# ucla-vision/xivo

Hardware: AMD Instinct MI355X
Metric: EKF updates/sec (state dim 250, 80 feats) @1 GPU; % MFMA roofline (higher is better)
Workload: dtype f64; 1 GPU; MH gating + UpdateJosephForm: state dim 250, 80 features (M=160), XIVO row sparsity, P/H/inn/R resident in HBM; filters_per_gpu=16384, global_batch=16384, parallelism=replicas x1 (no collective), pipeline=sparse-H (row-pair compressed H, whitened in-solve Joseph form), hand_over=dense H -> row-pair compressed rows every step, inside the timed region, route=sparse_in_solve, not_spd_filters=0

## Files before the change

### xivo_amd/csrc/trsm_lds_kernel.h

```cpp
#pragma once
#include <stdlib.h>
#include <stdio.h>

#include "mfma_util.h"

#ifndef XIVO_TRACE
#define XIVO_TRACE 0
#endif
#if XIVO_TRACE
__device__ unsigned long long xivo_trace_buf[512 * 32];
__device__ unsigned long long xivo_trace2_buf[128 * 16 * 4 * 16];
#define XTR(i) do { if (T4 && !WOUT && threadIdx.x == 0 && (blockIdx.x & 63) == 0 && (blockIdx.x >> 6) < 512) \
    xivo_trace_buf[(blockIdx.x >> 6) * 32 + (i)] = __builtin_amdgcn_s_memtime(); } while (0)
#define XTRP(i) do { if (FIXUP && threadIdx.x == 0 && (blockIdx.x & 63) == 0 && (blockIdx.x >> 6) < 512) \
    xivo_trace_buf[(blockIdx.x >> 6) * 32 + (i)] = __builtin_amdgcn_s_memtime(); } while (0)
#define XTR2(ph, slot) do { if (FIXUP && (threadIdx.x & 63) == 0 && (blockIdx.x & 63) == 0 && (blockIdx.x >> 6) < 128 && (ph) < 4 && (slot) < 16) \
    xivo_trace2_buf[(((blockIdx.x >> 6) * 16 + (threadIdx.x >> 6)) * 4 + (ph)) * 16 + (slot)] = __builtin_amdgcn_s_memtime(); } while (0)
extern "C" int xivo_hip_debug_read_trace(unsigned long long* out, int n) {
  return (int)hipMemcpyFromSymbol(out, HIP_SYMBOL(xivo_trace_buf), (size_t)n * sizeof(unsigned long long));
}
extern "C" int xivo_hip_debug_read_trace2(unsigned long long* out, int n) {
  return (int)hipMemcpyFromSymbol(out, HIP_SYMBOL(xivo_trace2_buf), (size_t)n * sizeof(unsigned long long));
}
#else
#define XTR(i) do {} while (0)
#define XTRP(i) do {} while (0)
#define XTR2(ph, slot) do {} while (0)
#endif

namespace xivo_hip {

namespace {

typedef unsigned int bufu2 __attribute__((ext_vector_type(2)));
__device__ __forceinline__ __amdgpu_buffer_rsrc_t buf_rsrc(const void* p) {
  return __builtin_amdgcn_make_buffer_rsrc(const_cast<void*>(p), 0, 0x7FFFFFFF, 0x00020000);
}
__device__ __forceinline__ double buf_ld(__amdgpu_buffer_rsrc_t r, unsigned voff, unsigned soff) {
  return __builtin_bit_cast(double, __builtin_amdgcn_raw_buffer_load_b64(r, voff, soff, 0));
}
__device__ __forceinline__ double buf_ld_once(__amdgpu_buffer_rsrc_t r, unsigned voff, unsigned soff) {
  return __builtin_bit_cast(double, __builtin_amdgcn_raw_buffer_load_b64(r, voff, soff, 0));
}
__device__ __forceinline__ void buf_st_f32(float v, __amdgpu_buffer_rsrc_t r, unsigned voff, unsigned soff) {
  __builtin_amdgcn_raw_buffer_store_b32(__builtin_bit_cast(unsigned, v), r, voff, soff, 0);
}
__device__ __forceinline__ void buf_st(double v, __amdgpu_buffer_rsrc_t r, unsigned voff, unsigned soff) {
  __builtin_amdgcn_raw_buffer_store_b64(__builtin_bit_cast(bufu2, v), r, voff, soff, 0);
}
__device__ __forceinline__ void buf_st_out(double v, __amdgpu_buffer_rsrc_t r, unsigned voff, unsigned soff) {
  __builtin_amdgcn_raw_buffer_store_b64(__builtin_bit_cast(bufu2, v), r, voff, soff, 0);
}

template <int NBM, bool SRC_REGS = false, bool NEG_OUT = false, bool FIXUP = false, bool YREGS = false, int NWV = 16>
__device__ __forceinline__ void sym_tiles_from_regs(const d4 (&X)[NBM], const d4 (&Wr)[NBM], double* sL, const double* __restrict__ Src, int ldsrc,
                                                    const double* __restrict__ Minit, int ldm, double* __restrict__ Out, int ldo,
                                                    int nb, int nwl, int jbp, bool live, int w, int wave, int lane) {
  const int li = lane & 15, lg = lane >> 4;
  const int nph = (nwl + jbp - 1) / jbp;
  const int bufsz = jbp * nb * 256;
  auto issue = [&](int p) {
    const int jb0 = p * jbp, nj = min(jbp, nwl - jb0);
    double* buf = sL + (p & 1) * bufsz;
    if (SRC_REGS) {
      if (live && w >= jb0 && w < jb0 + nj) {
        double* dst = buf + (w - jb0) * nb * 256 + lane;
#pragma unroll
        for (int mb = 0; mb < NBM; ++mb) {
          if (mb < nb) {
#pragma unroll
            for (int r = 0; r < 4; ++r) dst[(mb * 4 + r) * 64] = YREGS ? fma(2.0, Wr[mb][r], -X[mb][r]) : X[mb][r];
          }
        }
      }
      return;
    }
    for (int q = wave; q < nj * 2 * nb; q += NWV) {
      const int jl = q / (2 * nb), t = q - jl * 2 * nb;
      const double* src = Src + (16 * (jb0 + jl) + 2 * (lane & 7)) + (long)(8 * t + (lane >> 3)) * ldsrc;
      __builtin_amdgcn_global_load_lds((const __attribute__((address_space(1))) void*)src,
                                       (__attribute__((address_space(3))) void*)(buf + jl * nb * 256 + t * 128), 16, 0, 0);
    }
  };
  auto my_tiles = [&](int p) -> unsigned {
    unsigned todo = 0;
    if (!live || p >= nph) return todo;
    const int jb0 = p * jbp, nj = min(jbp, nwl - jb0);
    for (int jl = 0; jl < nj; ++jl) {
      int d = w - (jb0 + jl);
      if (d < 0) d += nwl;
      if (2 * d < nwl || (2 * d == nwl && w > jb0 + jl)) todo |= 1u << jl;
    }
    return todo;
  };
  const __amdgpu_buffer_rsrc_t rM = buf_rsrc(Minit), rO = buf_rsrc(Out);
  const unsigned vM = (unsigned)(li + lg * ldm) * 8u;
  const unsigned vO = (unsigned)(li + lg * ldo) * 8u, vOt = (unsigned)(lg + li * ldo) * 8u;
  auto load_m = [&](int jb, d4& acc) {
    const int ba = jb <= w ? w : jb, bb = jb <= w ? jb : w;
#pragma unroll
    for (int r = 0; r < 4; ++r)
      acc[r] = buf_ld_once(rM, vM, (unsigned)(16 * ba + (16 * bb + 4 * r) * ldm) * 8u);
  };
  issue(0);
  unsigned todo = my_tiles(0);
  d4 nxt = d4{0.0, 0.0, 0.0, 0.0};
  if (todo) load_m(__builtin_ctz(todo), nxt);
  for (int p = 0; p < nph; ++p) {
    XTRP(8 + 3 * p);
    asm volatile("s_waitcnt vmcnt(0)" ::: "memory");
    XTRP(9 + 3 * p);
    __syncthreads();
    XTRP(10 + 3 * p);
    XTR2(p, 0);
    int tslot = 2;
    const int jb0 = p * jbp;
    const double* buf = sL + (p & 1) * bufsz;
    if (FIXUP) {
      if (live && w >= jb0 && w < jb0 + min(jbp, nwl - jb0)) {
        double* dst = sL + (p & 1) * bufsz + (w - jb0) * nb * 256 + lane;
#pragma unroll
        for (int mb = 0; mb < NBM; ++mb) {
          if (mb < nb) {
#pragma unroll
            for (int r = 0; r < 4; ++r) dst[(mb * 4 + r) * 64] = fma(2.0, dst[(mb * 4 + r) * 64], -X[mb][r]);
          }
        }
      }
      lds_barrier();
    }
    XTR2(p, 1);
    bool fetch = p + 1 < nph;
    while (todo) {
      const int jl = __builtin_ctz(todo);
      todo &= todo - 1;
      const int jb = jb0 + jl;
      d4 acc = -nxt;
      if (fetch) { asm volatile("" : "+v"(acc[0]), "+v"(acc[1]), "+v"(acc[2]), "+v"(acc[3])); issue(p + 1); fetch = false; }
      if (todo) load_m(jb0 + __builtin_ctz(todo), nxt);
      const double* Bop = buf + jl * nb * 256 + lane;
      if (jb <= w) {
#pragma unroll
        for (int mb = 0; mb < NBM; ++mb) {
          if (mb < nb) {
#pragma unroll
            for (int r = 0; r < 4; ++r) acc = mfma(Bop[(mb * 4 + r) * 64], X[mb][r], acc);
          }
        }
      } else {
#pragma unroll
        for (int mb = 0; mb < NBM; ++mb) {
          if (mb < nb) {
#pragma unroll
            for (int r = 0; r < 4; ++r) acc = mfma(X[mb][r], Bop[(mb * 4 + r) * 64], acc);
          }
        }
      }
      XTR2(p, tslot); ++tslot;
      const int ba = jb <= w ? w : jb, bbk = jb <= w ? jb : w;
      const int a = 16 * ba + li, b = 16 * bbk + lg;
#pragma unroll
      for (int r = 0; r < 4; ++r) {
        const int bb = b + 4 * r;
        if (jb != w || a >= bb) {
          const double v = NEG_OUT ? -acc[r] : acc[r];
          buf_st_out(v, rO, vO, (unsigned)(16 * ba + (16 * bbk + 4 * r) * ldo) * 8u);
          if (a != bb) buf_st_out(v, rO, vOt, (unsigned)(16 * bbk + 4 * r + 16 * ba * ldo) * 8u);
        }
      }
      XTR2(p, tslot); ++tslot;
    }
    XTR2(p, 14);
    if (fetch) issue(p + 1);
    todo = my_tiles(p + 1);
    if (todo) load_m((p + 1) * jbp + __builtin_ctz(todo), nxt);
  }
  XTRP(8 + 3 * nph);
}

template <int NBM, int TF, int NWV = 16, int MINB = 1>
__global__ __launch_bounds__(64 * NWV, MINB) void trsm_lds_f64_kernel(TrsmArgs g) {
  constexpr int BLK = 16 * 17;
  constexpr int NT = 64 * NWV;
  static_assert(TF != 3, "TF == 3 (the round-2 expanded Joseph form) was removed in round 6");
  constexpr bool T4 = TF == 4 || TF == 5;
  constexpr bool WOUT = TF == 5;
  constexpr bool KEEPW = T4 && (NBM <= 6 || (NBM == 7 && NWV <= 12 && MINB <= 3));
  constexpr bool PACK = T4 && NBM > 10;
  extern __shared__ __attribute__((aligned(16))) double sL[];
  const int chunks = (g.Np + 16 * NWV - 1) / (16 * NWV);
  const int b = blockIdx.x;
  const int xcd = b & 7, slot = b >> 3;
  const int filt = (slot / chunks) * 8 + xcd;
  const int chunk = slot % chunks;
  if (filt >= g.batch) return;
  const int tid = threadIdx.x, lane = tid & 63, wave = __builtin_amdgcn_readfirstlane(tid >> 6);
  const int li = lane & 15, lg = lane >> 4;
  const int nb = g.Mp / 16;
  const double* __restrict__ LU = g.LU + (long)filt * g.strideLU;
  const double* __restrict__ invD = g.invD + (long)filt * g.strideInvD;
  const double* __restrict__ PHT = g.PHT + (long)filt * g.stridePHT;
  const long ld = g.ldlu;

  XTR(0);
  const int c0 = chunk * 16 * NWV + wave * 16;
  const bool live = c0 < g.Np;
  const __amdgpu_buffer_rsrc_t rPHT = buf_rsrc(PHT), rK = buf_rsrc(g.K + (long)filt * g.strideK),
                               rInn = buf_rsrc(g.fwd_only ? g.y + (long)filt * g.strideY : g.inn + (long)filt * g.strideInn);
  const unsigned vPHT = (unsigned)((c0 + li) + lg * g.ldpht) * 8u;
  const unsigned vK = (unsigned)((c0 + li) + lg * g.ldk) * 8u;
  d4 X[NBM];
  auto load_rhs = [&](int i0, int i1) {
#pragma unroll
    for (int i = 0; i < NBM; ++i) {
      if (i >= i0 && i < i1) {
        X[i] = d4{0.0, 0.0, 0.0, 0.0};
        if (live && i < nb) {
#pragma unroll
          for (int r = 0; r < 4; ++r) X[i][r] = buf_ld_once(rPHT, vPHT, (unsigned)((16 * i + 4 * r) * g.ldpht) * 8u);
        }
      }
    }
  };
  load_rhs(0, NBM);
  d4 Wk[KEEPW ? NBM : 1];
#pragma unroll
  for (int i = 0; i < (KEEPW ? NBM : 1); ++i) Wk[i] = d4{0.0, 0.0, 0.0, 0.0};

  const int nblk = nb * (nb + 1) / 2;
  constexpr bool DIAG = !PACK && T4;
  constexpr int CPY = (NBM * (NBM + 1) / 2 * 128 + NT - 1) / NT;
  constexpr int CPD = DIAG ? (NBM * 128 + NT - 1) / NT : 0;
  constexpr int CPB = 4;
  double* sD = sL + nblk * BLK;
#pragma unroll
  for (int u0 = 0; u0 < CPY + CPD; u0 += CPB) {
    d2 cv[CPB], cu[CPB];
#pragma unroll
    for (int q = 0; q < CPB; ++q) {
      const int u = u0 + q;
      cv[q] = d2{0.0, 0.0}; cu[q] = d2{0.0, 0.0};
      if (u < CPY) {
        const int e = tid + NT * u;
        if (e < nblk * 128) {
          const int t = e >> 7, w = e & 127;
          int i = 0;
          while ((i + 1) * (i + 2) / 2 <= t) ++i;
          const int k = t - i * (i + 1) / 2;
          const int r = (w & 7) * 2, c = w >> 3;
          cv[q] = *reinterpret_cast<const d2*>(i != k ? LU + (16 * i + r) + (long)(16 * k + c) * ld : invD + (long)k * 512 + r + 16 * c);
          if (PACK && i == k) { cu[q][0] = LU[(16 * k + c) + (long)(16 * k + r) * ld]; cu[q][1] = LU[(16 * k + c) + (long)(16 * k + r + 1) * ld]; }
        }
      } else if (u < CPY + CPD) {
        const int e = tid + NT * (u - CPY);
        if (e < nb * 128) {
          const int k = e >> 7, w = e & 127;
          cv[q] = *reinterpret_cast<const d2*>(LU + (16 * k + (w & 7) * 2) + (long)(16 * k + (w >> 3)) * ld);
        }
      }
    }
#pragma unroll
    for (int q = 0; q < CPB; ++q) {
      const int u = u0 + q;
      if (u < CPY) {
        const int e = tid + NT * u;
        if (e < nblk * 128) {
          const int t = e >> 7, w = e & 127;
          int i = 0;
          while ((i + 1) * (i + 2) / 2 <= t) ++i;
          const int k = t - i * (i + 1) / 2;
          const int r = (w & 7) * 2, c = w >> 3;
          d2 v = cv[q];
          if (PACK && i == k) { v[0] = r >= c ? v[0] : cu[q][0]; v[1] = r + 1 >= c ? v[1] : cu[q][1]; }
          sL[t * BLK + r + 17 * c] = v[0];
          sL[t * BLK + r + 1 + 17 * c] = v[1];
        }
      } else if (u < CPY + CPD) {
        const int e = tid + NT * (u - CPY);
        if (e < nb * 128) {
          const int k = e >> 7, w = e & 127;
          const int r = (w & 7) * 2, c = w >> 3;
          sD[k * BLK + r + 17 * c] = r >= c ? cv[q][0] : 0.0;
          sD[k * BLK + r + 1 + 17 * c] = r + 1 >= c ? cv[q][1] : 0.0;
        }
      }
    }
    __builtin_amdgcn_sched_barrier(0);
  }
  if (PACK) {
    for (int e = tid; e < nb * 16; e += NT) {
      const int k = e >> 4, c = e & 15;
      sL[(k * (k + 1) / 2 + k) * BLK + 16 + 17 * c] = LU[(16 * k + c) + (long)(16 * k + c) * ld];
    }
  }
  XTR(1);
  __syncthreads();
  XTR(2);
  if (!TF && !live) return;
  if (live) {
#pragma unroll
  for (int k = 0; k < NBM; ++k) {
    if (k < nb) {
      const double* Dk = sL + (k * (k + 1) / 2 + k) * BLK;
      d4 t = d4{0.0, 0.0, 0.0, 0.0};
#pragma unroll
      for (int s = 0; s < 4; ++s) {
        double a = Dk[li + 17 * (4 * s + lg)];
        if (PACK) a = li >= 4 * s + lg ? a : 0.0;
        t = mfma(a, X[k][s], t);
      }
      X[k] = t;
#pragma unroll
      for (int s = 0; s < 4; ++s) {
#pragma unroll
        for (int i = k + 1; i < NBM; ++i) {
          if (i < nb) {
            const double a = sL[(i * (i + 1) / 2 + k) * BLK + li + 17 * (4 * s + lg)];
            X[i] = mfma(-a, t[s], X[i]);
          }
        }
      }
    }
  }
  XTR(3);
  double part = 0.0;
  if (KEEPW) {
#pragma unroll
    for (int i = 0; i < NBM; ++i) Wk[i] = X[i];
  }
  if (T4 && !KEEPW) {
#pragma unroll
    for (int i = 0; i < NBM; ++i) {
      if (i < nb) {
#pragma unroll
        for (int r = 0; r < 4; ++r) buf_st(X[i][r], rK, vK, (unsigned)((16 * i + 4 * r) * g.ldk) * 8u);
      }
    }
  }
  XTR(4);
#pragma unroll
  for (int k = NBM - 1; k >= 0; --k) {
    if (k < nb && !g.fwd_only) {
      const double* Dk = sL + (k * (k + 1) / 2 + k) * BLK;
      d4 wk = d4{0.0, 0.0, 0.0, 0.0};
      if (KEEPW) wk = Wk[k];
      else if (T4) {
        if (k == nb - 1) wk = X[k];
        else {
#pragma unroll
          for (int r = 0; r < 4; ++r) wk[r] = buf_ld(rK, vK, (unsigned)((16 * k + 4 * r) * g.ldk) * 8u);
        }
      }
      d4 t = d4{0.0, 0.0, 0.0, 0.0};
#pragma unroll
      for (int s = 0; s < 4; ++s) {
        double a = Dk[(4 * s + lg) + 17 * li];
        if (PACK) a = 4 * s + lg >= li ? a : 0.0;
        t = mfma(a, X[k][s], t);
      }
      if (T4) {
        const double* Lk = PACK ? Dk : sD + k * BLK;
#pragma unroll
        for (int s2 = 0; s2 < 4; ++s2) {
          const int kk = 4 * s2 + lg;
          if (PACK) {
            const double a = Lk[kk > li ? li + 17 * kk : 16 + 17 * li];
            X[k] = mfma(kk >= li ? -a : 0.0, t[s2], X[k]);
          } else {
            X[k] = mfma(-Lk[kk + 17 * li], t[s2], X[k]);
          }
        }
#pragma unroll
        for (int r = 0; r < 4; ++r) part = fma(t[r], buf_ld(rInn, (unsigned)lg * 8u, (unsigned)(16 * k + 4 * r) * 8u), part);
      } else {
        X[k] = t;
      }
#pragma unroll
      for (int s = 0; s < 4; ++s) {
#pragma unroll
        for (int i = 0; i < k; ++i) {
          const double a = sL[(k * (k + 1) / 2 + i) * BLK + (4 * s + lg) + 17 * li];
          X[i] = mfma(-a, t[s], X[i]);
        }
      }
      if (T4) {
        if (WOUT) {
          const __amdgpu_buffer_rsrc_t rY = buf_rsrc(g.Yout + (long)filt * g.strideY2);
#pragma unroll
          for (int r = 0; r < 4; ++r) buf_st(wk[r] + X[k][r], rY, (unsigned)((c0 + li) + lg * g.ldy2) * 8u, (unsigned)((16 * k + 4 * r) * g.ldy2) * 8u);
        }
        X[k] = wk - X[k];
        __builtin_amdgcn_sched_barrier(0);
      }
    }
  }

  if (!T4) {
#pragma unroll
    for (int i = 0; i < NBM; ++i) {
      if (i < nb) {
#pragma unroll
        for (int r = 0; r < 4; ++r) {
          if (TF != 2) buf_st(X[i][r], rK, vK, (unsigned)((16 * i + 4 * r) * g.ldk) * 8u);
          part = fma(X[i][r], buf_ld(rInn, (unsigned)lg * 8u, (unsigned)(16 * i + 4 * r) * 8u), part);
        }
      }
    }
  }
  part += __shfl_xor(part, 16);
  part += __shfl_xor(part, 32);
  if (lg == 0) g.err[(long)filt * g.strideErr + c0 + li] = part;


  }
  if (!TF) return;

  XTR(5);
  __syncthreads();
  XTR(6);
  if (T4) {
    if (WOUT) {
      if (live) {
#pragma unroll
        for (int i = 0; i < NBM; ++i) {
          if (i < nb) {
#pragma unroll
            for (int r = 0; r < 4; ++r) buf_st(X[i][r], rK, vK, (unsigned)((16 * i + 4 * r) * g.ldk) * 8u);
          }
        }
      }
      return;
    }
    if (g.skip_status && g.skip_status[filt] != 0) return;
    double* Pio = g.T + (long)filt * g.strideT;
    if constexpr (KEEPW) sym_tiles_from_regs<NBM, true, true, false, true, NWV>(X, Wk, sL, nullptr, 0, Pio, g.ldt, Pio, g.ldt, nb, g.Np / 16, g.t_jbp,
                                                                 live, c0 >> 4, wave, lane);
    else sym_tiles_from_regs<NBM, false, true, true, false, NWV>(X, X, sL, g.K + (long)filt * g.strideK, g.ldk, Pio, g.ldt, Pio, g.ldt, nb, g.Np / 16, g.t_jbp,
                                                     live, c0 >> 4, wave, lane);
    return;
  }
  if (TF == 2) {
    if (g.skip_status && g.skip_status[filt] != 0) return;
    double* Pio = g.T + (long)filt * g.strideT;
    sym_tiles_from_regs<NBM, true, true, false, false, NWV>(X, X, sL, nullptr, 0, Pio, g.ldt, Pio, g.ldt, nb, g.Np / 16, g.t_jbp, live, c0 >> 4, wave, lane);
    return;
  }
  sym_tiles_from_regs<NBM, false, false, false, false, NWV>(X, X, sL, PHT, g.ldpht, g.Pm + (long)filt * g.stridePm, g.ldpm, g.T + (long)filt * g.strideT, g.ldt,
                           nb, g.Np / 16, g.t_jbp, live, c0 >> 4, wave, lane);
}

}

}
```

Before: 926,800 updates/s.

## Add whitened Joseph tile kernel that keeps D in registers and skips redundant tiles

Adds a dedicated whitened_tiles_from_stash routine for the non-KEEPW T4 path. It keeps the back-substituted values in registers (DREGS), so the solve no longer reloads W from K or forms W-X there. The routine computes the fixup in place, writing the difference to LDS and the reflected value to registers, and uses a group-based tile schedule in which waves skip earlier phases entirely. The FIXUP template flag is removed from sym_tiles_from_regs. The risks are higher register pressure and a changed tile-ownership and symmetry logic (jb<w, d mod nj) that could leave tiles uncovered if the schedule is wrong.

```diff
diff --git a/xivo_amd/csrc/trsm_lds_kernel.h b/xivo_amd/csrc/trsm_lds_kernel.h
--- a/xivo_amd/csrc/trsm_lds_kernel.h
+++ b/xivo_amd/csrc/trsm_lds_kernel.h
@@ -12,9 +12,9 @@
 __device__ unsigned long long xivo_trace2_buf[128 * 16 * 4 * 16];
 #define XTR(i) do { if (T4 && !WOUT && threadIdx.x == 0 && (blockIdx.x & 63) == 0 && (blockIdx.x >> 6) < 512) \
     xivo_trace_buf[(blockIdx.x >> 6) * 32 + (i)] = __builtin_amdgcn_s_memtime(); } while (0)
-#define XTRP(i) do { if (FIXUP && threadIdx.x == 0 && (blockIdx.x & 63) == 0 && (blockIdx.x >> 6) < 512) \
+#define XTRP(i) do { if (threadIdx.x == 0 && (blockIdx.x & 63) == 0 && (blockIdx.x >> 6) < 512) \
     xivo_trace_buf[(blockIdx.x >> 6) * 32 + (i)] = __builtin_amdgcn_s_memtime(); } while (0)
-#define XTR2(ph, slot) do { if (FIXUP && (threadIdx.x & 63) == 0 && (blockIdx.x & 63) == 0 && (blockIdx.x >> 6) < 128 && (ph) < 4 && (slot) < 16) \
+#define XTR2(ph, slot) do { if ((threadIdx.x & 63) == 0 && (blockIdx.x & 63) == 0 && (blockIdx.x >> 6) < 128 && (ph) < 4 && (slot) < 16) \
     xivo_trace2_buf[(((blockIdx.x >> 6) * 16 + (threadIdx.x >> 6)) * 4 + (ph)) * 16 + (slot)] = __builtin_amdgcn_s_memtime(); } while (0)
 extern "C" int xivo_hip_debug_read_trace(unsigned long long* out, int n) {
   return (int)hipMemcpyFromSymbol(out, HIP_SYMBOL(xivo_trace_buf), (size_t)n * sizeof(unsigned long long));
@@ -52,7 +52,7 @@
   __builtin_amdgcn_raw_buffer_store_b64(__builtin_bit_cast(bufu2, v), r, voff, soff, 0);
 }
 
-template <int NBM, bool SRC_REGS = false, bool NEG_OUT = false, bool FIXUP = false, bool YREGS = false, int NWV = 16>
+template <int NBM, bool SRC_REGS = false, bool NEG_OUT = false, bool YREGS = false, int NWV = 16>
 __device__ __forceinline__ void sym_tiles_from_regs(const d4 (&X)[NBM], const d4 (&Wr)[NBM], double* sL, const double* __restrict__ Src, int ldsrc,
                                                     const double* __restrict__ Minit, int ldm, double* __restrict__ Out, int ldo,
                                                     int nb, int nwl, int jbp, bool live, int w, int wave, int lane) {
@@ -101,6 +101,97 @@
 #pragma unroll
     for (int r = 0; r < 4; ++r)
       acc[r] = buf_ld_once(rM, vM, (unsigned)(16 * ba + (16 * bb + 4 * r) * ldm) * 8u);
+  };
+  issue(0);
+  unsigned todo = my_tiles(0);
+  d4 nxt = d4{0.0, 0.0, 0.0, 0.0};
+  if (todo) load_m(__builtin_ctz(todo), nxt);
+  for (int p = 0; p < nph; ++p) {
+    asm volatile("s_waitcnt vmcnt(0)" ::: "memory");
+    __syncthreads();
+    const int jb0 = p * jbp;
+    const double* buf = sL + (p & 1) * bufsz;
+    bool fetch = p + 1 < nph;
+    while (todo) {
+      const int jl = __builtin_ctz(todo);
+      todo &= todo - 1;
+      const int jb = jb0 + jl;
+      d4 acc = -nxt;
+      if (fetch) { asm volatile("" : "+v"(acc[0]), "+v"(acc[1]), "+v"(acc[2]), "+v"(acc[3])); issue(p + 1); fetch = false; }
+      if (todo) load_m(jb0 + __builtin_ctz(todo), nxt);
+      const double* Bop = buf + jl * nb * 256 + lane;
+      if (jb <= w) {
+#pragma unroll
+        for (int mb = 0; mb < NBM; ++mb) {
+          if (mb < nb) {
+#pragma unroll
+            for (int r = 0; r < 4; ++r) acc = mfma(Bop[(mb * 4 + r) * 64], X[mb][r], acc);
+          }
+        }
+      } else {
+#pragma unroll
+        for (int mb = 0; mb < NBM; ++mb) {
+          if (mb < nb) {
+#pragma unroll
+            for (int r = 0; r < 4; ++r) acc = mfma(X[mb][r], Bop[(mb * 4 + r) * 64], acc);
+          }
+        }
+      }
+      const int ba = jb <= w ? w : jb, bbk = jb <= w ? jb : w;
+      const int a = 16 * ba + li, b = 16 * bbk + lg;
+#pragma unroll
+      for (int r = 0; r < 4; ++r) {
+        const int bb = b + 4 * r;
+        if (jb != w || a >= bb) {
+          const double v = NEG_OUT ? -acc[r] : acc[r];
+          buf_st_out(v, rO, vO, (unsigned)(16 * ba + (16 * bbk + 4 * r) * ldo) * 8u);
+          if (a != bb) buf_st_out(v, rO, vOt, (unsigned)(16 * bbk + 4 * r + 16 * ba * ldo) * 8u);
+        }
+      }
+    }
+    if (fetch) issue(p + 1);
+    todo = my_tiles(p + 1);
+    if (todo) load_m((p + 1) * jbp + __builtin_ctz(todo), nxt);
+  }
+}
+
+template <int NBM, int NWV>
+__device__ __forceinline__ void whitened_tiles_from_stash(d4 (&X)[NBM], double* sL, const double* __restrict__ Src, int ldsrc,
+                                                          double* __restrict__ Pio, int ldp, int nb, int nwl, int jbp, bool live,
+                                                          int w, int wave, int lane) {
+  const int li = lane & 15, lg = lane >> 4;
+  const int nph = (nwl + jbp - 1) / jbp;
+  const int bufsz = jbp * nb * 256;
+  const int gw = w / jbp;
+  auto issue = [&](int p) {
+    const int jb0 = p * jbp, nj = min(jbp, nwl - jb0);
+    double* buf = sL + (p & 1) * bufsz;
+    for (int q = wave; q < nj * 2 * nb; q += NWV) {
+      const int jl = q / (2 * nb), t = q - jl * 2 * nb;
+      const double* src = Src + (16 * (jb0 + jl) + 2 * (lane & 7)) + (long)(8 * t + (lane >> 3)) * ldsrc;
+      __builtin_amdgcn_global_load_lds((const __attribute__((address_space(1))) void*)src,
+                                       (__attribute__((address_space(3))) void*)(buf + jl * nb * 256 + t * 128), 16, 0, 0);
+    }
+  };
+  auto my_tiles = [&](int p) -> unsigned {
+    if (!live || p >= nph || gw > p) return 0u;
+    const int jb0 = p * jbp, nj = min(jbp, nwl - jb0);
+    if (gw < p) return (1u << nj) - 1u;
+    unsigned todo = 0;
+    for (int jl = 0; jl < nj; ++jl) {
+      int d = w - (jb0 + jl);
+      if (d < 0) d += nj;
+      if (2 * d < nj || (2 * d == nj && w > jb0 + jl)) todo |= 1u << jl;
+    }
+    return todo;
+  };
+  const __amdgpu_buffer_rsrc_t rP = buf_rsrc(Pio);
+  const unsigned vP = (unsigned)(li + lg * ldp) * 8u, vPt = (unsigned)(lg + li * ldp) * 8u;
+  auto load_m = [&](int jb, d4& acc) {
+    const int ba = jb <= w ? w : jb, bb = jb <= w ? jb : w;
+#pragma unroll
+    for (int r = 0; r < 4; ++r)
+      acc[r] = buf_ld_once(rP, vP, (unsigned)(16 * ba + (16 * bb + 4 * r) * ldp) * 8u);
   };
   issue(0);
   unsigned todo = my_tiles(0);
@@ -116,19 +207,22 @@
     int tslot = 2;
     const int jb0 = p * jbp;
     const double* buf = sL + (p & 1) * bufsz;
-    if (FIXUP) {
-      if (live && w >= jb0 && w < jb0 + min(jbp, nwl - jb0)) {
-        double* dst = sL + (p & 1) * bufsz + (w - jb0) * nb * 256 + lane;
-#pragma unroll
-        for (int mb = 0; mb < NBM; ++mb) {
-          if (mb < nb) {
-#pragma unroll
-            for (int r = 0; r < 4; ++r) dst[(mb * 4 + r) * 64] = fma(2.0, dst[(mb * 4 + r) * 64], -X[mb][r]);
-          }
-        }
-      }
-      lds_barrier();
-    }
+    if (live && gw == p) {
+      double* dst = sL + (p & 1) * bufsz + (w - jb0) * nb * 256 + lane;
+#pragma unroll
+      for (int mb = 0; mb < NBM; ++mb) {
+        if (mb < nb) {
+#pragma unroll
+          for (int r = 0; r < 4; ++r) {
+            const double wv = dst[(mb * 4 + r) * 64];
+            const double v = wv - X[mb][r];
+            X[mb][r] = fma(2.0, wv, -v);
+            dst[(mb * 4 + r) * 64] = v;
+          }
+        }
+      }
+    }
+    lds_barrier();
     XTR2(p, 1);
     bool fetch = p + 1 < nph;
     while (todo) {
@@ -139,7 +233,7 @@
       if (fetch) { asm volatile("" : "+v"(acc[0]), "+v"(acc[1]), "+v"(acc[2]), "+v"(acc[3])); issue(p + 1); fetch = false; }
       if (todo) load_m(jb0 + __builtin_ctz(todo), nxt);
       const double* Bop = buf + jl * nb * 256 + lane;
-      if (jb <= w) {
+      if (jb < w) {
 #pragma unroll
         for (int mb = 0; mb < NBM; ++mb) {
           if (mb < nb) {
@@ -163,9 +257,9 @@
       for (int r = 0; r < 4; ++r) {
         const int bb = b + 4 * r;
         if (jb != w || a >= bb) {
-          const double v = NEG_OUT ? -acc[r] : acc[r];
-          buf_st_out(v, rO, vO, (unsigned)(16 * ba + (16 * bbk + 4 * r) * ldo) * 8u);
-          if (a != bb) buf_st_out(v, rO, vOt, (unsigned)(16 * bbk + 4 * r + 16 * ba * ldo) * 8u);
+          const double v = -acc[r];
+          buf_st_out(v, rP, vP, (unsigned)(16 * ba + (16 * bbk + 4 * r) * ldp) * 8u);
+          if (a != bb) buf_st_out(v, rP, vPt, (unsigned)(16 * bbk + 4 * r + 16 * ba * ldp) * 8u);
         }
       }
       XTR2(p, tslot); ++tslot;
@@ -187,6 +281,7 @@
   constexpr bool WOUT = TF == 5;
   constexpr bool KEEPW = T4 && (NBM <= 6 || (NBM == 7 && NWV <= 12 && MINB <= 3));
   constexpr bool PACK = T4 && NBM > 10;
+  constexpr bool DREGS = T4 && !KEEPW && !WOUT;
   extern __shared__ __attribute__((aligned(16))) double sL[];
   const int chunks = (g.Np + 16 * NWV - 1) / (16 * NWV);
   const int b = blockIdx.x;
@@ -344,7 +439,7 @@
       const double* Dk = sL + (k * (k + 1) / 2 + k) * BLK;
       d4 wk = d4{0.0, 0.0, 0.0, 0.0};
       if (KEEPW) wk = Wk[k];
-      else if (T4) {
+      else if (T4 && !DREGS) {
         if (k == nb - 1) wk = X[k];
         else {
 #pragma unroll
@@ -389,7 +484,7 @@
 #pragma unroll
           for (int r = 0; r < 4; ++r) buf_st(wk[r] + X[k][r], rY, (unsigned)((c0 + li) + lg * g.ldy2) * 8u, (unsigned)((16 * k + 4 * r) * g.ldy2) * 8u);
         }
-        X[k] = wk - X[k];
+        if (!DREGS) X[k] = wk - X[k];
         __builtin_amdgcn_sched_barrier(0);
       }
     }
@@ -433,19 +528,18 @@
     }
     if (g.skip_status && g.skip_status[filt] != 0) return;
     double* Pio = g.T + (long)filt * g.strideT;
-    if constexpr (KEEPW) sym_tiles_from_regs<NBM, true, true, false, true, NWV>(X, Wk, sL, nullptr, 0, Pio, g.ldt, Pio, g.ldt, nb, g.Np / 16, g.t_jbp,
+    if constexpr (KEEPW) sym_tiles_from_regs<NBM, true, true, true, NWV>(X, Wk, sL, nullptr, 0, Pio, g.ldt, Pio, g.ldt, nb, g.Np / 16, g.t_jbp,
                                                                  live, c0 >> 4, wave, lane);
-    else sym_tiles_from_regs<NBM, false, true, true, false, NWV>(X, X, sL, g.K + (long)filt * g.strideK, g.ldk, Pio, g.ldt, Pio, g.ldt, nb, g.Np / 16, g.t_jbp,
-                                                     live, c0 >> 4, wave, lane);
+    else whitened_tiles_from_stash<NBM, NWV>(X, sL, g.K + (long)filt * g.strideK, g.ldk, Pio, g.ldt, nb, g.Np / 16, g.t_jbp, live, c0 >> 4, wave, lane);
     return;
   }
   if (TF == 2) {
     if (g.skip_status && g.skip_status[filt] != 0) return;
     double* Pio = g.T + (long)filt * g.strideT;
-    sym_tiles_from_regs<NBM, true, true, false, false, NWV>(X, X, sL, nullptr, 0, Pio, g.ldt, Pio, g.ldt, nb, g.Np / 16, g.t_jbp, live, c0 >> 4, wave, lane);
+    sym_tiles_from_regs<NBM, true, true, false, NWV>(X, X, sL, nullptr, 0, Pio, g.ldt, Pio, g.ldt, nb, g.Np / 16, g.t_jbp, live, c0 >> 4, wave, lane);
     return;
   }
-  sym_tiles_from_regs<NBM, false, false, false, false, NWV>(X, X, sL, PHT, g.ldpht, g.Pm + (long)filt * g.stridePm, g.ldpm, g.T + (long)filt * g.strideT, g.ldt,
+  sym_tiles_from_regs<NBM, false, false, false, NWV>(X, X, sL, PHT, g.ldpht, g.Pm + (long)filt * g.stridePm, g.ldpm, g.T + (long)filt * g.strideT, g.ldt,
                            nb, g.Np / 16, g.t_jbp, live, c0 >> 4, wave, lane);
 }
 
```

Result: faster. 945,900 updates/s (median of 6 runs) (+2.1%).
